# skyplane-project/skyplane

Hardware: NVIDIA H100
Metric: chunk-pipeline GB/s (raw input) (higher is better)
Workload: dtype u8/u32

## Files before the change

### skyplane_b200/csrc/md5.cuh

```cuda
#pragma once
#include <stdint.h>
#include "xxh32.cuh"
#include <type_traits>
#include <utility>

#ifndef SKY_MD5_SLOTS
#define SKY_MD5_SLOTS 4
#endif

namespace sky {

struct Md5State {
    uint32_t a, b, c, d;
};

__device__ __forceinline__ void md5_init(Md5State &s) {
    s.a = 0x67452301u;
    s.b = 0xefcdab89u;
    s.c = 0x98badcfeu;
    s.d = 0x10325476u;
}

__device__ __forceinline__ uint32_t md5_am(uint32_t a, uint32_t m, uint32_t one) {
    uint32_t r;
    asm("mad.lo.u32 %0, %1, %2, %3;" : "=r"(r) : "r"(m), "r"(one), "r"(a));
    return r;
}
__device__ __forceinline__ uint32_t md5_one() {
    uint32_t eq, lane;
    asm("mov.u32 %0, %%lanemask_eq;" : "=r"(eq));
    asm("mov.u32 %0, %%laneid;" : "=r"(lane));
    return eq >> lane;
}
#define SKY_MD5_STEP(FN, a, b, c, d, m, k, s)                      \
    {                                                              \
        uint32_t t_ = FN(b, c, d) + md5_am(a, (m), one) + (k);     \
        a = b + __funnelshift_l(t_, t_, s);                        \
    }
#define SKY_F(b, c, d) ((d) ^ ((b) & ((c) ^ (d))))
#define SKY_G(b, c, d) ((c) ^ ((d) & ((b) ^ (c))))
#define SKY_H(b, c, d) ((b) ^ (c) ^ (d))
#define SKY_I(b, c, d) ((c) ^ ((b) | ~(d)))

// ... 85 lines not shown

template <int kSlot>
__device__ __forceinline__ void cp_async_block(bool pred, uint32_t lane_ring, const uint8_t *gptr) {
    asm volatile(
        "{\n\t.reg .pred p;\n\t"
        "setp.ne.b32 p, %2, 0;\n\t"
        "@p cp.async.cg.shared.global [%0+%3], [%1], 16;\n\t"
        "@p cp.async.cg.shared.global [%0+%4], [%1+16], 16;\n\t"
        "@p cp.async.cg.shared.global [%0+%5], [%1+32], 16;\n\t"
        "@p cp.async.cg.shared.global [%0+%6], [%1+48], 16;\n\t}" ::"r"(lane_ring),
        "l"(gptr), "r"((uint32_t)pred), "n"(kSlot * 2048), "n"(kSlot * 2048 + 512), "n"(kSlot * 2048 + 1024),
        "n"(kSlot * 2048 + 1536)
        : "memory");
}
__device__ __forceinline__ void cp_async_commit() { asm volatile("cp.async.commit_group;\n" ::: "memory"); }
template <int N>
__device__ __forceinline__ void cp_async_wait() {
    asm volatile("cp.async.wait_group %0;\n" ::"n"(N) : "memory");
}

template <class F, int... I>
__device__ __forceinline__ void md5_unroll_(F &&f, std::integer_sequence<int, I...>) {
    (f(std::integral_constant<int, I>()), ...);
}
template <int N, class F>
__device__ __forceinline__ void md5_unroll(F &&f) {
    md5_unroll_(f, std::make_integer_sequence<int, N>());
}

struct Md5NoGate {
    __device__ __forceinline__ void operator()(uint64_t, bool) const {}
};

template <bool kXxh = false, class Gate = Md5NoGate>
__device__ __forceinline__ uint32_t md5_warp(uint32_t *ring, const uint8_t *src, uint64_t len, bool active, uint8_t *out,
                                             unsigned lane, Gate gate = Gate()) {
    constexpr int kSlots = SKY_MD5_SLOTS;
    static_assert(kSlots >= 2 && (kSlots & (kSlots - 1)) == 0 && 1024 % kSlots == 0, "SKY_MD5_SLOTS: a power of two, 2..1024");
    constexpr bool kGated = !std::is_same<Gate, Md5NoGate>::value;
    const uint32_t nfull = active ? (uint32_t)(len >> 6) : 0;
    const uint32_t wmax = __reduce_max_sync(0xffffffffu, nfull);
    const uint32_t trips = (wmax + (kSlots - 1)) & ~(uint32_t)(kSlots - 1);
    Md5State st;
    md5_init(st);
    Md5State fin = st;
    XxhState xs, xfin;
    if constexpr (kXxh) {
        xxh_init(xs);
        xfin = xs;
    }
    const uint32_t *lring = ring + lane * 4;
    const uint32_t lring_s = (uint32_t)__cvta_generic_to_shared(lring);
    const uint32_t one = md5_one();

    gate(0, active && len > 0);
    md5_unroll<kSlots - 1>([&](auto sc) {
        constexpr int s = decltype(sc)::value;
        cp_async_block<s>((uint32_t)s < nfull, lring_s, src + s * 64);
        cp_async_commit();
    });
    auto load_words = [&](uint32_t (&w)[16], int cs) {
#pragma unroll
        for (int q = 0; q < 4; q++) {
            const uint4 v = *reinterpret_cast<const uint4 *>(lring + (cs * 4 + q) * 128);
            w[4 * q + 0] = v.x;
            w[4 * q + 1] = v.y;
            w[4 * q + 2] = v.z;
            w[4 * q + 3] = v.w;
        }
    };
    uint32_t w[2][16];
    cp_async_wait<kSlots - 2>();
    load_words(w[0], 0);
    const uint8_t *pf_src = src + (kSlots - 1) * 64;
    auto blocks = [&](uint32_t i) {
        md5_unroll<kSlots>([&](auto uc) {
            constexpr int u = decltype(uc)::value;
            constexpr int ps = (u + kSlots - 1) & (kSlots - 1);
            constexpr int ns = (u + 1) & (kSlots - 1);
            uint32_t a = st.a, b = st.b, c = st.c, d = st.d;
            const uint32_t(&wu)[16] = w[u & 1];
            auto stripe = [&](int q) {
                if constexpr (kXxh) xxh_stripe(xs, wu[4 * q], wu[4 * q + 1], wu[4 * q + 2], wu[4 * q + 3]);
            };
            md5_round<0>(a, b, c, d, wu, one);
            stripe(0);
            cp_async_block<ps>(i + u + (kSlots - 1) < nfull, lring_s, pf_src + u * 64);
            md5_round<1>(a, b, c, d, wu, one);
            stripe(1);
            cp_async_commit();
            cp_async_wait<kSlots - 2>();
            md5_round<2>(a, b, c, d, wu, one);
            stripe(2);
            load_words(w[(u + 1) & 1], ns);
            md5_round<3>(a, b, c, d, wu, one);
            stripe(3);
            st.a += a;
            st.b += b;
            st.c += c;
            st.d += d;
            if (i + u < nfull) {
                fin = st;
                if constexpr (kXxh) xfin = xs;
            }
        });
        pf_src += kSlots * 64;
    };
    if constexpr (kGated) {
        for (uint32_t base = 0; base < trips; base += 1024) {
            gate((base >> 10) + 1, (uint64_t)(base + 1024) * 64 < len);
            const uint32_t iend = min(base + 1024, trips);
            for (uint32_t i = base; i < iend; i += kSlots) blocks(i);
        }
    } else {
        for (uint32_t i = 0; i < trips; i += kSlots) blocks(i);
    }
    cp_async_wait<0>();
    st = fin;
    uint32_t xxh = 0;
    if (active) {
        const uint32_t rem = (uint32_t)(len & 63);
        const uint8_t *tp = src + ((uint64_t)nfull << 6);
        uint32_t tw[32];
#pragma unroll
        for (int k = 0; k < 32; k++) tw[k] = 0;
        for (uint32_t k = 0; k < rem; k++) tw[k >> 2] |= (uint32_t)tp[k] << (8 * (k & 3));
        if constexpr (kXxh) {
            xs = xfin;
            const uint32_t nstripes = rem >> 4;
            for (uint32_t q = 0; q < nstripes; q++) xxh_stripe(xs, tw[4 * q], tw[4 * q + 1], tw[4 * q + 2], tw[4 * q + 3]);
            uint32_t h = xxh_merge(xs, len);
            for (uint32_t k = 4 * nstripes; k < (rem >> 2); k++) h = xxh_word(h, tw[k]);
            for (uint32_t k = rem & ~3u; k < rem; k++) h = xxh_byte(h, (tw[k >> 2] >> (8 * (k & 3))) & 0xffu);
            xxh = xxh_avalanche(h);
        }
        tw[rem >> 2] |= 0x80u << (8 * (rem & 3));
        const bool two = rem >= 56;
        const uint64_t bits = len << 3;
        tw[two ? 30 : 14] = (uint32_t)bits;
        tw[two ? 31 : 15] = (uint32_t)(bits >> 32);
        for (int t = 0; t < (two ? 2 : 1); t++) {
            uint32_t w[16];
#pragma unroll
            for (int k = 0; k < 16; k++) w[k] = tw[16 * t + k];
            md5_block(st, w, one);
        }
        uint4 dg = make_uint4(st.a, st.b, st.c, st.d);
        *reinterpret_cast<uint4 *>(out) = dg;
    }
// ... 5 lines not shown
```

### skyplane_b200/csrc/skychunk.cu

```cuda

#include <cuda_runtime.h>
#include <stdint.h>
#include <stdio.h>
#include <string.h>

#include <algorithm>
#include <memory>
#include <new>
#include <numeric>
#include <string>
#include <utility>
#include <vector>

#include "../../include/skychunk.h"
#include "frame.cuh"
#include "lz4.cuh"
#include "lz4dec.cuh"
#include "lz4hc.cuh"
#include "lz4verify.cuh"
#include "md5.cuh"
#include "secretbox.cuh"

namespace sky {

#ifndef SKY_PARSERS
#define SKY_PARSERS 12
#endif
constexpr int kParsers = SKY_PARSERS;
constexpr int kProbers = 2;
constexpr int kWarps = kProbers + kParsers;
constexpr int kThreads = kWarps * 32;
#ifndef SKY_RING_EXTRA
#define SKY_RING_EXTRA 2
#endif
constexpr int kRing = kParsers + SKY_RING_EXTRA;
constexpr int kMd5WarpsPerCta = 4;
constexpr uint32_t kRingBytes = SKY_MD5_SLOTS * 2048;
constexpr int kCtasPerSm = 2;
constexpr uint64_t kMaxChunkBlocks = 1ull << 21;

struct Ctl {
    uint64_t in_full;
    uint64_t full[kRing], empty[kRing];
    BlockDesc desc[2];
    uint32_t claim;
    volatile uint32_t block_end_seq;
    volatile uint32_t nseg;
    volatile uint32_t seg_hit[4];
    uint32_t raw, last_lits, tail_off;
    uint64_t data;
    uint32_t size;
    PendingChecksum pend;
};
constexpr uint32_t kInOff = 0;
constexpr uint32_t kTabOff = kInOff + kInBytes;
constexpr uint32_t kRingOff = kTabOff + kTableBytes;
constexpr uint32_t kRecOff = kRingOff + kRing * (uint32_t)sizeof(SegSlot);
constexpr uint32_t kPlanOff = kRecOff + kMaxSegs * (uint32_t)sizeof(SegRec);
constexpr uint32_t kCtlOff = kPlanOff + kMaxSegs * (uint32_t)sizeof(SegPlan);
constexpr uint32_t kSmemBytes = (kCtlOff + (uint32_t)sizeof(Ctl) + 127u) & ~127u;
static_assert(kSmemBytes <= 232448 / 2 - 1024, "two CTAs per SM need <= 112.5 KiB each: lower SKY_PARSERS or SKY_LZ4_ENTRIES");
static_assert(kEntries % 128 == 0, "SKY_LZ4_ENTRIES must be a multiple of 128");
static_assert(kMd5WarpsPerCta * kRingBytes <= kInBytes, "the MD5 rings live in the block buffer of a digest CTA");
static_assert(sizeof(SegSlot) % 16 == 0 && sizeof(SegRec) == 16 && sizeof(SegPlan) == 16, "layout");

template <int kId>
__device__ __forceinline__ void bar_arrive() { asm volatile("bar.arrive %0, 64;" ::"n"(kId) : "memory"); }
template <int kId>
__device__ __forceinline__ void bar_wait() { asm volatile("bar.sync %0, 64;" ::"n"(kId) : "memory"); }

template <bool kXxh, bool kBlkChk>
__device__ __forceinline__ void fused_body(const Params &p) {
    extern __shared__ __align__(128) uint8_t smem[];
    const unsigned warp = threadIdx.x >> 5, lane = threadIdx.x & 31;
    uint8_t *in = smem + kInOff;
    uint32_t *tab = reinterpret_cast<uint32_t *>(smem + kTabOff);
    SegSlot *ring = reinterpret_cast<SegSlot *>(smem + kRingOff);
    SegRec *recs = reinterpret_cast<SegRec *>(smem + kRecOff);
    SegPlan *plans = reinterpret_cast<SegPlan *>(smem + kPlanOff);
    Ctl *ctl = reinterpret_cast<Ctl *>(smem + kCtlOff);
    uint32_t smem_s = smem_u32(smem);
    asm volatile("" : "+r"(smem_s));

    const bool do_md5 = (p.flags & SKY_F_MD5) != 0, do_lz4 = (p.flags & SKY_F_LZ4) != 0;
    if (warp == 0 && lane == 0) {
        mbar_init(&ctl->in_full, 1);
        for (int i = 0; i < kRing; i++) {
            mbar_init(&ctl->full[i], 1);
            mbar_init(&ctl->empty[i], 1);
        }
        ctl->claim = 0;
        if constexpr (kBlkChk) ctl->pend.data = nullptr;
        asm volatile("fence.mbarrier_init.release.cluster;" ::: "memory");
    }
    __syncthreads();

    if (do_md5 && blockIdx.x < p.n_md5_ctas) {
        if (warp < kMd5WarpsPerCta) {
            for (uint32_t g = warp * p.n_md5_ctas + blockIdx.x; g < p.n_groups; g += p.n_md5_ctas * kMd5WarpsPerCta) {
                const uint32_t c = p.md5_order[g * 32 + lane];
                const bool active = c != 0xffffffffu;
                const uint8_t *src = nullptr;
                uint64_t len = 0;
                if (active) {
                    src = p.chunks[c].src;
                    len = p.chunks[c].len;
                }
                const uint32_t x = md5_warp<kXxh>(reinterpret_cast<uint32_t *>(in + warp * kRingBytes), src, len, active,
                                                  p.md5_out + (size_t)(active ? c : 0) * 16, lane);
                if constexpr (kXxh) {
                    if (active) p.xxh_out[c] = x;
                }
                __syncwarp();
            }
        }
        if (!do_lz4) return;
        __syncthreads();
    }
    if (!do_lz4) return;

    uint8_t *scratch = p.scratch + (size_t)blockIdx.x * kScratchBytes;
    uint32_t gseq = 0;
    uint32_t batches_done = 0;
    uint32_t my_seq = 0;
    bool have_claim = false;
    uint32_t in_phase = 0;
    constexpr unsigned kSumWarp = kWarps - 1;
    for (uint32_t it = 0;; it++) {
        BlockDesc *dsc = &ctl->desc[it & 1];
        if (warp == 0 && lane == 0) {
            claim_block(p, dsc);
            ctl->block_end_seq = 0xffffffffu;
            ctl->nseg = 0;
        }
        __syncthreads();
        if (!dsc->valid) {
            if constexpr (kBlkChk) {
                if (warp == kSumWarp) run_pending(&ctl->pend, lane);
            }
            break;
        }
        const uint8_t *src = dsc->src;
        const uint32_t L = dsc->L;

        if (warp < kProbers) {
            if (warp == 0) {
                if (lane == 0) load_block(in, src, L, &ctl->in_full);
                uint4 *t4 = reinterpret_cast<uint4 *>(tab);
                const uint4 z = make_uint4(0, 0, 0, 0);
#pragma unroll 4
                for (uint32_t k = lane; k < kEntries / 4; k += 32) t4[k] = z;
                __syncwarp();
            }
            mbar_wait(&ctl->in_full, in_phase);
            in_phase ^= 1;
            uint32_t nseg = 0;
            if (L >= kMfLimit + 1) {
                const uint32_t mflimit = L - kMfLimit;
                uint32_t seg_pos = 0, slog = 0;
                while (seg_pos <= mflimit) {
                    if (nseg >= 2) {
                        const bool h = ctl->seg_hit[(nseg - 2) & 3u] != 0u;
                        slog = h ? 0u : min(slog + 1u, kMaxStepLog);
                    }
                    const uint32_t si = gseq % kRing, ph = (gseq / kRing) & 1u;
                    SegSlot *slot = ring + si;
// ... 215 lines not shown
    p.status[c] = st;
}

struct DecRowGate {
    const uint32_t *flags;
    __device__ __forceinline__ void operator()(uint64_t row, bool wants) const {
        unsigned ns = 128;
        for (;;) {
            const bool ready = !wants || ld_relaxed32(flags + row) != 0;
            if (__all_sync(kFull, ready)) break;
            __nanosleep(ns);
            if (ns < 4096) ns <<= 1;
        }
        asm volatile("fence.acq_rel.gpu;" ::: "memory");
    }
};

__global__ void __launch_bounds__(512, 1) sky_decode_kernel(const DecParams p) {
    extern __shared__ __align__(128) uint8_t smem[];
    const unsigned warp = threadIdx.x >> 5, lane = threadIdx.x & 31;
    if (warp < kMd5WarpsPerCta) {
        const uint32_t md5_slots = gridDim.x * kMd5WarpsPerCta;
        for (uint32_t g = warp * gridDim.x + blockIdx.x; g < p.n_groups; g += md5_slots) {
            const uint32_t c = p.md5_order[g * 32 + lane];
            const bool active = c != 0xffffffffu;
            const uint8_t *src = nullptr;
            uint64_t len = 0;
            DecRowGate gate{nullptr};
            if (active) {
                src = p.chunks[c].out;
                len = p.chunks[c].raw_len;
                gate.flags = p.blk_done + p.chunks[c].blk_base;
            }
            const uint32_t x = md5_warp<true>(reinterpret_cast<uint32_t *>(smem + warp * kRingBytes), src, len, active,
                                              p.md5_out + (size_t)(active ? c : 0) * 16, lane, gate);
            if (active) {
                const int32_t s = settle_status(*reinterpret_cast<volatile int32_t *>(p.status + c));
                if (s != kDecOk) p.status[c] = s;
                else if ((p.chunks[c].checks & kChkContent) && x != p.chunks[c].content_xxh) atomicCAS(p.status + c, kDecOk, kDecChecksum);
            }
            __syncwarp();
        }
    }
    for (uint32_t c, j; claim_row_major(p.counter, p.n_chunks, p.rows, lane, c, j);) {
        const DecChunk cd = p.chunks[c];
        if (j >= cd.nblk) continue;
        int32_t st = *reinterpret_cast<volatile int32_t *>(p.status + c);
        const uint64_t pos = (uint64_t)j * kBlock;
        const uint32_t want = (uint32_t)min((uint64_t)kBlock, cd.raw_len - pos);
        if (cd.linked) {
            if (lane == 0) {
                unsigned ns = 64;
                while (ld_acquire32(p.dec_done + c) < j) {
                    __nanosleep(ns);
                    if (ns < 2048) ns <<= 1;
                }
            }
            __syncwarp();
            st = *reinterpret_cast<volatile int32_t *>(p.status + c);
        }
        if (block_may_run(st, j)) {
            const DecBlock b = p.blocks[cd.blk_base + j];
            const uint32_t sz = b.word & 0x7FFFFFFFu;
            if ((cd.checks & kChkBlock) && xxh32_warp(cd.frame + b.off, sz, lane) != b.chk) {
                st = kDecChecksum;
            } else if (b.word & 0x80000000u) {
                st = sz != want ? kDecLayout : kDecOk;
                if (st == kDecOk) warp_copy(cd.out + pos, cd.frame + b.off, sz, lane);
// ... 175 lines not shown

static thread_local std::string g_err;

#define CK(ctx, call)                                                                      \
    do {                                                                                   \
        cudaError_t e_ = (call);                                                           \
        if (e_ != cudaSuccess) {                                                           \
            char b_[512];                                                                  \
            snprintf(b_, sizeof b_, "%s -> %s (%s:%d)", #call, cudaGetErrorString(e_), __FILE__, __LINE__); \
            if (ctx) (ctx)->err = b_;                                                      \
            g_err = b_;                                                                    \
            return SKY_E_CUDA;                                                             \
        }                                                                                  \
    } while (0)

static int build_slot(sky_ctx *ctx, Slot &s, bool slabs) {
    const size_t nc = ctx->max_chunks, ng = (nc + 31) / 32 * 32;
    CK(ctx, cudaStreamCreateWithFlags(s.stream.put(), cudaStreamNonBlocking));
    CK(ctx, cudaEventCreate(s.ev_k0.put()));
    CK(ctx, cudaEventCreate(s.ev_k1.put()));
    CK(ctx, cudaEventCreate(s.ev_res.put()));
    CK(ctx, cudaEventCreateWithFlags(s.ev_h2d.put(), cudaEventDisableTiming));
    CK(ctx, cudaEventCreateWithFlags(s.ev_d2h.put(), cudaEventDisableTiming));
    BatchMeta &m = s.meta;
    CK(ctx, cudaMallocHost(m.h_desc.put(), nc * sizeof(ChunkDesc)));
    CK(ctx, cudaMalloc(m.d_desc.put(), nc * sizeof(ChunkDesc)));
    CK(ctx, cudaMallocHost(m.h_order.put(), ng * sizeof(uint32_t)));
    CK(ctx, cudaMalloc(m.d_order.put(), ng * sizeof(uint32_t)));
    CK(ctx, cudaMallocHost(m.h_chain.put(), nc * sizeof(uint64_t)));
    CK(ctx, cudaMalloc(m.d_chain.put(), nc * sizeof(uint64_t)));
    CK(ctx, m.outlen.alloc(nc));
    CK(ctx, m.md5.alloc(nc * 16));
    CK(ctx, cudaMalloc(m.xxh.put(), nc * sizeof(uint32_t)));
    CK(ctx, cudaMalloc(m.counters.put(), 64));
    CK(ctx, cudaMalloc(m.scratch.put(), (size_t)ctx->sm_count * kCtasPerSm * kScratchBytes));
    if (slabs) {
        cudaError_t e = cudaMalloc(s.d_in.put(), ctx->in_cap);
        if (e == cudaSuccess) e = cudaMalloc(s.d_out.put(), ctx->out_cap);
        if (e != cudaSuccess) { g_err = ctx->err = std::string("cudaMalloc(slab): ") + cudaGetErrorString(e); return SKY_E_NOMEM; }
    }
    return SKY_OK;
}

static int alloc_dec(sky_ctx *ctx, DecodeArrays &d) {
    if (d.d_chunks) return SKY_OK;
    const size_t nc = ctx->max_chunks;
    DecodeArrays a;
    CK(ctx, cudaMallocHost(a.h_chunks.put(), nc * sizeof(DecChunk)));
    CK(ctx, cudaMalloc(a.d_chunks.put(), nc * sizeof(DecChunk)));
    CK(ctx, cudaMallocHost(a.h_status.put(), nc * sizeof(int32_t)));
    CK(ctx, cudaMalloc(a.d_status.put(), nc * sizeof(int32_t)));
    CK(ctx, cudaMalloc(a.d_dec_done.put(), nc * sizeof(uint32_t)));
    d = std::move(a);
    return SKY_OK;
}

static int alloc_hc(sky_ctx *ctx, HcArrays &h) {
    if (h.scratch) return SKY_OK;
    HcArrays a;
    CK(ctx, cudaMalloc(a.scratch.put(), (size_t)ctx->sm_count * kHcLinkedScratchBytes));
    CK(ctx, cudaStreamCreateWithFlags(a.md5_stream.put(), cudaStreamNonBlocking));
    CK(ctx, cudaEventCreateWithFlags(a.ev_fork.put(), cudaEventDisableTiming));
    CK(ctx, cudaEventCreateWithFlags(a.ev_join.put(), cudaEventDisableTiming));
    h = std::move(a);
    return SKY_OK;
}

// ... 297 lines not shown
    (linked ? sky_verify_linked_kernel : sky_verify_kernel)<<<ctx->sm_count * 2, kVerifyThreads, 0, st>>>(p);
    CK(ctx, cudaGetLastError());
    (linked ? sky_verify_linked_settle_kernel : sky_verify_settle_kernel)<<<n, kRepairWarps * 32, 0, st>>>(p);
    CK(ctx, cudaGetLastError());
    ctx->launches += 3;
    return SKY_OK;
}

static int launch_batch(sky_ctx *ctx, Slot &s, cudaStream_t st, cudaStream_t meta_st, uint32_t n, const uint8_t *d_src,
                        const uint64_t *src_off, const uint64_t *src_len, uint8_t *d_dst, const uint64_t *dst_off, uint32_t flags) {
    if ((flags & (SKY_F_LZ4 | SKY_F_MD5)) == 0) flags |= SKY_F_LZ4 | SKY_F_MD5;
    if (flags & SKY_F_CHECKSUM) flags |= SKY_F_MD5;
    const bool xxh = (flags & SKY_F_CHECKSUM) != 0, bc = (flags & SKY_F_BLOCK_CHECKSUM) != 0;
    if (flags & SKY_F_HC) {
        const int hrc = alloc_hc(ctx, s.hc);
        if (hrc != SKY_OK) return hrc;
    }
    BatchMeta &m = s.meta;
    uint32_t rows;
    int rc = batch_geometry(n, src_len, rows, [&](uint32_t i, uint32_t nblk) {
        m.h_desc[i] = ChunkDesc{d_src + src_off[i], d_dst + dst_off[i], src_len[i], nblk};
        m.h_chain[i] = kFrameHeaderBytes;
    });
    if (rc != SKY_OK) return rc;
    const uint32_t ng = fill_md5_order(m.h_order, n, src_len);

    CK(ctx, cudaMemcpyAsync(m.d_desc, m.h_desc, n * sizeof(ChunkDesc), cudaMemcpyHostToDevice, meta_st));
    CK(ctx, cudaMemcpyAsync(m.d_order, m.h_order, ng * 32 * sizeof(uint32_t), cudaMemcpyHostToDevice, meta_st));
    CK(ctx, cudaMemcpyAsync(m.d_chain, m.h_chain, n * sizeof(uint64_t), cudaMemcpyHostToDevice, meta_st));
    if (meta_st != st) {
        CK(ctx, cudaEventRecord(s.ev_h2d, meta_st));
        CK(ctx, cudaStreamWaitEvent(st, s.ev_h2d, 0));
    }
    CK(ctx, cudaMemsetAsync(m.counters, 0, 64, st));
    memset(m.outlen.h, 0, n * sizeof(uint64_t));
    memset(m.md5.h, 0, (size_t)n * 16);

    Params p;
    p.chunks = m.d_desc;
    p.md5_order = m.d_order;
    p.chain = m.d_chain;
    p.out_len = m.outlen.d;
    p.md5_out = m.md5.d;
    p.counters = m.counters;
    p.scratch = m.scratch;
    p.n_chunks = n;
    p.n_groups = ng;
    const uint32_t grid = (uint32_t)ctx->sm_count * kCtasPerSm;
    p.n_md5_ctas = (flags & SKY_F_MD5) ? std::min(grid, std::max((ng + kMd5WarpsPerCta - 1) / kMd5WarpsPerCta,
                                                                 std::min(ng, (uint32_t)ctx->sm_count / 4))) : 0;
    p.rows = rows;
    p.flags = flags;
    p.xxh_out = m.xxh;
    CK(ctx, cudaEventRecord(s.ev_k0, st));
    if (flags & SKY_F_HC) {
        HcArrays &h = s.hc;
        const bool md5 = (flags & SKY_F_MD5) != 0;
        if (md5) {
            CK(ctx, cudaEventRecord(h.ev_fork, st));
            CK(ctx, cudaStreamWaitEvent(h.md5_stream, h.ev_fork, 0));
            Params pm = p;
            pm.flags = SKY_F_MD5;
            if (xxh) sky_fused_xxh_kernel<<<grid, kThreads, kSmemBytes, h.md5_stream>>>(pm);
            else sky_fused_kernel<<<grid, kThreads, kSmemBytes, h.md5_stream>>>(pm);
            CK(ctx, cudaGetLastError());
            CK(ctx, cudaEventRecord(h.ev_join, h.md5_stream));
            ctx->launches++;
// ... 225 lines not shown
    DecodeArrays &d = s.dec;
    uint64_t nblk_total = 0;
    uint32_t rows;
    rc = batch_geometry(n, raw_len, rows, [&](uint32_t i, uint32_t nblk) {
        d.h_chunks[i] = DecChunk{d_frames + frame_off[i], d_out + out_off[i], frame_len[i], raw_len[i], nblk_total, nblk, 0};
        nblk_total += nblk;
    });
    if (rc == SKY_OK) rc = grow_block_table(ctx, st, d.table, nblk_total + 1);
    if (rc != SKY_OK) return rc;
    BatchMeta &m = s.meta;
    CK(ctx, cudaMemcpyAsync(d.d_chunks, d.h_chunks, n * sizeof(DecChunk), cudaMemcpyHostToDevice, st));
    CK(ctx, cudaMemsetAsync(m.counters, 0, 64, st));
    CK(ctx, cudaMemsetAsync(d.d_dec_done, 0, n * sizeof(uint32_t), st));
    CK(ctx, cudaMemsetAsync(d.d_status, 0, n * sizeof(int32_t), st));
    CK(ctx, cudaMemsetAsync(d.table.done, 0, (nblk_total + 1) * sizeof(uint32_t), st));
    const uint32_t ng = fill_md5_order(m.h_order, n, raw_len);
    CK(ctx, cudaMemcpyAsync(m.d_order, m.h_order, ng * 32 * sizeof(uint32_t), cudaMemcpyHostToDevice, st));
    memset(m.md5.h, 0, (size_t)n * 16);
    DecParams p;
    p.chunks = d.d_chunks;
    p.blocks = d.table.blocks;
    p.status = d.d_status;
    p.dec_done = d.d_dec_done;
    p.counter = m.counters;
    p.blk_done = d.table.done;
    p.md5_order = m.d_order;
    p.md5_out = m.md5.d;
    p.n_chunks = n;
    p.n_groups = ng;
    p.rows = rows;
    CK(ctx, cudaEventRecord(s.ev_k0, st));
    sky_frame_index_kernel<<<(n + 127) / 128, 128, 0, st>>>(p);
    CK(ctx, cudaGetLastError());
    sky_decode_kernel<<<ctx->sm_count, 512, kMd5WarpsPerCta * kRingBytes, st>>>(p);
    CK(ctx, cudaGetLastError());
    CK(ctx, cudaEventRecord(s.ev_k1, st));
    ctx->launches += 2;
    CK(ctx, cudaMemcpyAsync(d.h_status, d.d_status, n * sizeof(int32_t), cudaMemcpyDeviceToHost, st));
    return SKY_OK;
}

int sky_decode_device(sky_ctx *ctx, uint32_t n, const void *d_frames, const uint64_t *frame_off, const uint64_t *frame_len,
                      void *d_out, const uint64_t *out_off, const uint64_t *raw_len, void *stream, int32_t *status, uint8_t *md5,
                      float *kernel_ms) {
    if (!ctx || n == 0 || !d_frames || !frame_off || !frame_len || !out_off || !raw_len) return SKY_E_INVALID;
    if (n > ctx->max_chunks) return SKY_E_CAPACITY;
    if (reinterpret_cast<uintptr_t>(d_out) & 15) return SKY_E_INVALID;
    for (uint32_t i = 0; i < n; i++) {
        if (out_off[i] & 15) return SKY_E_INVALID;
        if (raw_len[i] && !d_out) return SKY_E_INVALID;
    }
    CK(ctx, cudaSetDevice(ctx->device));
    Slot &s = ctx->slots[0];
    if (s.ticket.busy) return SKY_E_BUSY;
    cudaStream_t st = stream ? (cudaStream_t)stream : s.stream;
    int rc = launch_decode(ctx, s, st, n, (const uint8_t *)d_frames, frame_off, frame_len, (uint8_t *)d_out, out_off, raw_len);
    if (rc != SKY_OK) return rc;
    CK(ctx, cudaStreamSynchronize(st));
    if (status) memcpy(status, s.dec.h_status, n * sizeof(int32_t));
    if (md5) memcpy(md5, s.meta.md5.h, (size_t)n * 16);
    if (kernel_ms) CK(ctx, cudaEventElapsedTime(kernel_ms, s.ev_k0, s.ev_k1));
    return SKY_OK;
}

static int decode_raw(sky_ctx *ctx, Slot &s, uint32_t n, const void *const *payload, const uint64_t *payload_len, void *const *dst,
                      const uint64_t *raw_len, bool e2ee, int32_t *status, uint8_t *md5, float *kernel_ms) {
    std::vector<uint64_t> off(n), box_off(n), msg_len(payload_len, payload_len + n), md5_len(n);
// ... 53 lines not shown
    for (uint32_t i = 0; i < n; i++) {
        if (!frames[i] || (raw_len[i] && !dst[i])) return SKY_E_INVALID;
        f_off[i] = fp;
        o_off[i] = op;
        fp += round16(frame_len[i]);
        op += round16(raw_len[i]);
    }
    if (fp > ctx->out_cap || op > ctx->in_cap) return SKY_E_CAPACITY;
    if (e2ee) {
        int rc = launch_open(ctx, s, n, frames, frame_len, f_off.data(), s.d_out, f_off.data(), f_len.data());
        if (rc != SKY_OK) return rc;
    } else {
        for (uint32_t i = 0; i < n; i++)
            CK(ctx, cudaMemcpyAsync(s.d_out + f_off[i], frames[i], frame_len[i], cudaMemcpyHostToDevice, s.stream));
    }
    int rc = sky_decode_device(ctx, n, s.d_out, f_off.data(), f_len.data(), s.d_in, o_off.data(), raw_len, s.stream, status, md5, kernel_ms);
    if (rc != SKY_OK) return rc;
    if (e2ee) {
        for (uint32_t i = 0; i < n; i++)
            if (s.box.h_status[i] != 0 || frame_len[i] < (uint64_t)kBoxOverhead) {
                s.dec.h_status[i] = SKY_D_AUTH;
                if (status) status[i] = SKY_D_AUTH;
            }
    }
    for (uint32_t i = 0; i < n; i++)
        if (raw_len[i] && s.dec.h_status[i] == 0)
            CK(ctx, cudaMemcpyAsync(dst[i], s.d_in + o_off[i], raw_len[i], cudaMemcpyDeviceToHost, s.stream));
    CK(ctx, cudaStreamSynchronize(s.stream));
    return SKY_OK;
}

uint64_t sky_launch_count(const sky_ctx *ctx) { return ctx ? ctx->launches : 0; }

}
```

### skyplane_b200/native.py

```python
from __future__ import annotations

import ctypes
from pathlib import Path
from typing import Optional, Sequence

_PKG = Path(__file__).resolve().parent
LIB_PATH = _PKG / "libskychunk.so"

SKY_OK = 0
SKY_E_INVALID, SKY_E_NOGPU, SKY_E_CUDA, SKY_E_CAPACITY, SKY_E_BUSY, SKY_E_TICKET, SKY_E_NOMEM, SKY_E_NOKEY = -1, -2, -3, -4, -5, -6, -7, -8
F_LZ4, F_MD5, F_E2EE, F_HC, F_CHECKSUM, F_BLOCK_CHECKSUM = 1, 2, 16, 32, 64, 128
F_VERIFY = 1 << 12
F_LINKED = 1 << 13
CHECKSUM_BYTES = 4
BLOCK_BYTES = 65536
HC_LEVEL_SHIFT = 8
HC_LEVEL_MASK = 0xF << HC_LEVEL_SHIFT
HC_MIN_LEVEL, HC_DEFAULT_LEVEL, HC_MAX_LEVEL = 3, 5, 9
BOX_OVERHEAD = 40
D_OK, D_BAD_HEADER, D_CORRUPT, D_SIZE, D_UNSUPPORTED, D_LAYOUT, D_TRUNCATED, D_AUTH, D_CHECKSUM = 0, -1, -2, -3, -4, -5, -6, -7, -8
D_MISMATCH = -9
D_NAMES = {0: "ok", -1: "bad frame header", -2: "corrupt block", -3: "size mismatch", -4: "unsupported frame feature",
           -5: "unexpected block layout", -6: "truncated frame", -7: "box authentication failed", -8: "checksum mismatch",
           -9: "frame decodes to other bytes"}

ABI_SYMBOLS = (
    "sky_strerror", "sky_last_error", "sky_abi_version", "sky_device_count", "sky_device_pci_bus_id", "sky_kernel_config", "sky_frame_bound",
    "sky_ctx_create", "sky_ctx_destroy", "sky_pinned_alloc", "sky_pinned_free",
    "sky_submit", "sky_wait", "sky_wait_verify", "sky_set_e2ee_key", "sky_box_bound", "sky_process_device", "sky_verify_device",
    "sky_decode_device", "sky_decode",
    "sky_device_alloc", "sky_device_free", "sky_memcpy_h2d", "sky_memcpy_d2h", "sky_launch_count",
)


# ... 126 lines not shown
    if level < HC_MIN_LEVEL:
        if hc:
            raise ValueError(f"compression_level {level} is the fast compressor: the high-ratio mode takes {HC_MIN_LEVEL}..{HC_MAX_LEVEL}")
        return 0
    return hc_level_flag(level)


def frame_bound(n: int) -> int:
    return int(lib().sky_frame_bound(n))


def frame_need(n: int, checksum: bool = False, block_checksum: bool = False) -> int:
    blocks = -(-n // BLOCK_BYTES)
    return frame_bound(n) + (CHECKSUM_BYTES if checksum else 0) + (CHECKSUM_BYTES * blocks if block_checksum else 0)


_DECODE_ONLY_SUBMIT = ((F_HC, "F_HC"), (HC_LEVEL_MASK, "a high-ratio level"), (F_CHECKSUM, "F_CHECKSUM"),
                       (F_BLOCK_CHECKSUM, "F_BLOCK_CHECKSUM"), (F_VERIFY, "F_VERIFY"), (F_LINKED, "F_LINKED"))


def check_decode_flags(flags: int) -> int:
    for bit, name in _DECODE_ONLY_SUBMIT:
        if flags & bit:
            raise ValueError(f"decode does not take {name}: it is a sender option (flags {flags:#x})")
    if flags & ~(F_LZ4 | F_MD5 | F_E2EE):
        raise ValueError(f"decode does not know flag bits {flags & ~(F_LZ4 | F_MD5 | F_E2EE):#x}")
    return flags


def round16(x: int) -> int:
    return (x + 15) & ~15


def device_count() -> int:
    n = ctypes.c_int(0)
    rc = lib().sky_device_count(ctypes.byref(n))
    if rc != SKY_OK:
        return 0
    return n.value


class PinnedBuffer:

    def __init__(self, nbytes: int):
        self.nbytes = int(nbytes)
        self.addr = lib().sky_pinned_alloc(self.nbytes)
        if not self.addr:
            raise SkyChunkError(SKY_E_NOMEM, "sky_pinned_alloc failed (no CUDA device?)")
        self._arr = (ctypes.c_ubyte * max(1, self.nbytes)).from_address(self.addr)
        self.view = memoryview(self._arr).cast("B")[: self.nbytes]

    def close(self):
        if self.addr:
            self.view.release()
            del self._arr
            lib().sky_pinned_free(self.addr)
            self.addr = None

    def __del__(self):
        try:
            self.close()
        except Exception:
            pass


class Context:
# ... 46 lines not shown
        A = ctypes.c_void_p * n
        U = ctypes.c_uint64 * n
        args = (A(*src_addrs), U(*src_lens), A(*dst_addrs) if dst_addrs is not None else None, U(*dst_caps) if dst_caps is not None else None, nonces)
        if nonces is not None and len(nonces) != 24 * n:
            raise ValueError("need 24 nonce bytes per chunk")
        t = ctypes.c_uint64(0)
        self._check(lib().sky_submit(self._h, n, args[0], args[1], args[2], args[3], flags, nonces, ctypes.byref(t)))
        self._inflight[t.value] = (n, args)
        return t.value

    def wait(self, ticket: int):
        n, _keep = self._inflight.pop(ticket)
        out = (ctypes.c_uint64 * n)()
        md5 = (ctypes.c_ubyte * (16 * n))()
        ms = ctypes.c_float(0)
        self._check(lib().sky_wait(self._h, ticket, out, md5, ctypes.byref(ms)))
        raw = bytes(md5)
        return list(out), [raw[16 * i : 16 * i + 16] for i in range(n)], ms.value

    def wait_verify(self, ticket: int):
        n, _keep = self._inflight[ticket]
        out = (ctypes.c_uint64 * n)()
        md5 = (ctypes.c_ubyte * (16 * n))()
        ver = (ctypes.c_int32 * n)()
        ms = ctypes.c_float(0)
        self._check(lib().sky_wait_verify(self._h, ticket, out, md5, ver, ctypes.byref(ms)))
        del self._inflight[ticket]
        raw = bytes(md5)
        return list(out), [raw[16 * i : 16 * i + 16] for i in range(n)], list(ver), ms.value

    def process_device(self, d_src: int, src_off: Sequence[int], src_len: Sequence[int], d_dst: int, dst_off: Sequence[int],
                       dst_cap: Sequence[int], flags: int = 0, stream: int = 0):
        n = len(src_len)
        U = ctypes.c_uint64 * n
        out = U()
        md5 = (ctypes.c_ubyte * (16 * n))()
        ms = ctypes.c_float(0)
        self._check(
            lib().sky_process_device(self._h, n, d_src, U(*src_off), U(*src_len), d_dst, U(*dst_off), U(*dst_cap), flags,
                                     stream or None, out, md5, ctypes.byref(ms))
        )
        raw = bytes(md5)
        return list(out), [raw[16 * i : 16 * i + 16] for i in range(n)], ms.value

    def verify_device(self, d_src: int, src_off: Sequence[int], src_len: Sequence[int], d_frames: int, frame_off: Sequence[int],
                      frame_len: Sequence[int], frame_cap: Optional[Sequence[int]] = None, content_xxh: Optional[Sequence[int]] = None,
                      flags: int = 0, stream: int = 0):
        n = len(src_len)
        U = ctypes.c_uint64 * n
        fl = U(*frame_len)
        st = (ctypes.c_int32 * n)()
        ms = ctypes.c_float(0)
        self._check(lib().sky_verify_device(self._h, n, d_src, U(*src_off), U(*src_len), d_frames, U(*frame_off), fl,
                                            U(*frame_cap) if frame_cap is not None else None,
                                            (ctypes.c_uint32 * n)(*content_xxh) if content_xxh is not None else None, flags,
                                            stream or None, st, ctypes.byref(ms)))
        return list(st), list(fl), ms.value

    def decode_device(self, d_frames: int, frame_off: Sequence[int], frame_len: Sequence[int], d_out: int, out_off: Sequence[int],
                      raw_len: Sequence[int], stream: int = 0):
        n = len(frame_len)
        U = ctypes.c_uint64 * n
        st = (ctypes.c_int32 * n)()
        md5 = (ctypes.c_ubyte * (16 * n))()
        ms = ctypes.c_float(0)
        self._check(lib().sky_decode_device(self._h, n, d_frames, U(*frame_off), U(*frame_len), d_out, U(*out_off), U(*raw_len),
                                            stream or None, st, md5, ctypes.byref(ms)))
        raw = bytes(md5)
        return list(st), [raw[16 * i : 16 * i + 16] for i in range(n)], ms.value

    def decode(self, frame_addrs: Sequence[int], frame_lens: Sequence[int], dst_addrs: Optional[Sequence[int]], raw_lens: Sequence[int],
               flags: int = 0):
        check_decode_flags(flags)
        n = len(frame_addrs)
        A = ctypes.c_void_p * n
        U = ctypes.c_uint64 * n
# ... 30 lines not shown
```

Measured before the change: 155.9.

## Deepen MD5 cp.async ring, add chain-aware LZ4 claim throttling and tracing

Raises the default MD5 prefetch ring from 4 to 8 slots and decouples the unroll factor (fixed at 4) from ring depth, prefetching a full ring ahead with runtime slot offsets. The decode kernel keeps its own 4-slot ring. Adds a default-on SKY_CHAIN_WAIT scheme where digest CTAs publish a per-SM estimated MD5 chain end time and LZ4 claimers sleep to avoid finishing far ahead of the MD5 tail. This also grows the counters buffer. Other changes are optional trace instrumentation and Python host-side array marshaling via array.array. The added sleeping heuristic uses a hard-coded cycles-per-block constant and risks idling compressor warps.

Result: faster. 162.7 (median of 6 runs) (+4.4%).

```diff
diff --git a/skyplane_b200/csrc/md5.cuh b/skyplane_b200/csrc/md5.cuh
--- a/skyplane_b200/csrc/md5.cuh
+++ b/skyplane_b200/csrc/md5.cuh
@@ -5,10 +5,49 @@
 #include <utility>
 
 #ifndef SKY_MD5_SLOTS
-#define SKY_MD5_SLOTS 4
+#define SKY_MD5_SLOTS 8
 #endif
 
 namespace sky {
+
+#ifdef SKY_MD5_TRACE
+constexpr int kTraceGroups = 256, kTraceStamps = 512, kTraceEvery = 1024;
+struct Md5TraceStamp {
+    uint64_t t;
+    uint32_t clk;
+    uint32_t wait;
+};
+struct Md5Trace {
+    uint32_t smid, warpid, cta, stamps;
+    uint64_t t0, t1;
+    uint32_t c0, c1, wait, blocks;
+    Md5TraceStamp s[kTraceStamps];
+};
+__device__ Md5Trace g_md5_trace[kTraceGroups];
+__device__ __forceinline__ uint64_t trace_globaltimer() {
+    uint64_t t;
+    asm volatile("mov.u64 %0, %%globaltimer;" : "=l"(t));
+    return t;
+}
+__device__ __forceinline__ uint32_t trace_clock() {
+    uint32_t c;
+    asm volatile("mov.u32 %0, %%clock;" : "=r"(c));
+    return c;
+}
+__device__ __forceinline__ uint32_t trace_smid() {
+    uint32_t s;
+    asm volatile("mov.u32 %0, %%smid;" : "=r"(s));
+    return s;
+}
+__device__ __forceinline__ uint32_t trace_warpid() {
+    uint32_t w;
+    asm volatile("mov.u32 %0, %%warpid;" : "=r"(w));
+    return w;
+}
+#define SKY_MD5_TRACE_PARAM , Md5Trace *trace = nullptr
+#else
+#define SKY_MD5_TRACE_PARAM
+#endif
 
 struct Md5State {
     uint32_t a, b, c, d;
@@ -160,15 +199,16 @@
     __device__ __forceinline__ void operator()(uint64_t, bool) const {}
 };
 
-template <bool kXxh = false, class Gate = Md5NoGate>
+template <bool kXxh = false, class Gate = Md5NoGate, int kSlots = SKY_MD5_SLOTS>
 __device__ __forceinline__ uint32_t md5_warp(uint32_t *ring, const uint8_t *src, uint64_t len, bool active, uint8_t *out,
-                                             unsigned lane, Gate gate = Gate()) {
-    constexpr int kSlots = SKY_MD5_SLOTS;
-    static_assert(kSlots >= 2 && (kSlots & (kSlots - 1)) == 0 && 1024 % kSlots == 0, "SKY_MD5_SLOTS: a power of two, 2..1024");
+                                             unsigned lane, Gate gate = Gate() SKY_MD5_TRACE_PARAM) {
+    constexpr int kUnroll = 4;
+    static_assert((kSlots & (kSlots - 1)) == 0 && kSlots % kUnroll == 0 && 1024 % kSlots == 0,
+                  "the MD5 ring: a power of two, a multiple of 4 and at most 1024 blocks");
     constexpr bool kGated = !std::is_same<Gate, Md5NoGate>::value;
     const uint32_t nfull = active ? (uint32_t)(len >> 6) : 0;
     const uint32_t wmax = __reduce_max_sync(0xffffffffu, nfull);
-    const uint32_t trips = (wmax + (kSlots - 1)) & ~(uint32_t)(kSlots - 1);
+    const uint32_t trips = (wmax + (kUnroll - 1)) & ~(uint32_t)(kUnroll - 1);
     Md5State st;
     md5_init(st);
     Md5State fin = st;
@@ -180,17 +220,27 @@
     const uint32_t *lring = ring + lane * 4;
     const uint32_t lring_s = (uint32_t)__cvta_generic_to_shared(lring);
     const uint32_t one = md5_one();
+#ifdef SKY_MD5_TRACE
+    uint32_t wait_cycles = 0;
+    if (trace && lane == 0) {
+        trace->smid = trace_smid();
+        trace->warpid = trace_warpid();
+        trace->cta = blockIdx.x;
+        trace->t0 = trace_globaltimer();
+        trace->c0 = trace_clock();
+    }
+#endif
 
     gate(0, active && len > 0);
-    md5_unroll<kSlots - 1>([&](auto sc) {
+    md5_unroll<kSlots>([&](auto sc) {
         constexpr int s = decltype(sc)::value;
         cp_async_block<s>((uint32_t)s < nfull, lring_s, src + s * 64);
         cp_async_commit();
     });
-    auto load_words = [&](uint32_t (&w)[16], int cs) {
+    auto load_words = [&](uint32_t (&w)[16], uint32_t so) {
 #pragma unroll
         for (int q = 0; q < 4; q++) {
-            const uint4 v = *reinterpret_cast<const uint4 *>(lring + (cs * 4 + q) * 128);
+            const uint4 v = *reinterpret_cast<const uint4 *>(lring + so / 4 + q * 128);
             w[4 * q + 0] = v.x;
             w[4 * q + 1] = v.y;
             w[4 * q + 2] = v.z;
@@ -198,14 +248,13 @@
         }
     };
     uint32_t w[2][16];
-    cp_async_wait<kSlots - 2>();
+    cp_async_wait<kSlots - 1>();
     load_words(w[0], 0);
-    const uint8_t *pf_src = src + (kSlots - 1) * 64;
+    const uint8_t *pf_src = src + kSlots * 64;
     auto blocks = [&](uint32_t i) {
-        md5_unroll<kSlots>([&](auto uc) {
+        const uint32_t so = (i & (kSlots - 1)) * 2048, so_next = ((i + kUnroll) & (kSlots - 1)) * 2048;
+        md5_unroll<kUnroll>([&](auto uc) {
             constexpr int u = decltype(uc)::value;
-            constexpr int ps = (u + kSlots - 1) & (kSlots - 1);
-            constexpr int ns = (u + 1) & (kSlots - 1);
             uint32_t a = st.a, b = st.b, c = st.c, d = st.d;
             const uint32_t(&wu)[16] = w[u & 1];
             auto stripe = [&](int q) {
@@ -213,14 +262,20 @@
             };
             md5_round<0>(a, b, c, d, wu, one);
             stripe(0);
-            cp_async_block<ps>(i + u + (kSlots - 1) < nfull, lring_s, pf_src + u * 64);
+            cp_async_block<u>(i + u + kSlots < nfull, lring_s + so, pf_src + u * 64);
             md5_round<1>(a, b, c, d, wu, one);
             stripe(1);
             cp_async_commit();
-            cp_async_wait<kSlots - 2>();
+#ifdef SKY_MD5_TRACE
+            const uint32_t wait_from = trace_clock();
+#endif
+            cp_async_wait<kSlots - 1>();
+#ifdef SKY_MD5_TRACE
+            wait_cycles += trace_clock() - wait_from;
+#endif
             md5_round<2>(a, b, c, d, wu, one);
             stripe(2);
-            load_words(w[(u + 1) & 1], ns);
+            load_words(w[(u + 1) & 1], u + 1 < kUnroll ? so + (u + 1) * 2048 : so_next);
             md5_round<3>(a, b, c, d, wu, one);
             stripe(3);
             st.a += a;
@@ -232,17 +287,33 @@
                 if constexpr (kXxh) xfin = xs;
             }
         });
-        pf_src += kSlots * 64;
+        pf_src += kUnroll * 64;
     };
     if constexpr (kGated) {
         for (uint32_t base = 0; base < trips; base += 1024) {
             gate((base >> 10) + 1, (uint64_t)(base + 1024) * 64 < len);
             const uint32_t iend = min(base + 1024, trips);
-            for (uint32_t i = base; i < iend; i += kSlots) blocks(i);
+            for (uint32_t i = base; i < iend; i += kUnroll) blocks(i);
         }
     } else {
-        for (uint32_t i = 0; i < trips; i += kSlots) blocks(i);
-    }
+        for (uint32_t i = 0; i < trips; i += kUnroll) {
+            blocks(i);
+#ifdef SKY_MD5_TRACE
+            const uint32_t done = i + kUnroll;
+            if (trace && lane == 0 && done % kTraceEvery == 0 && done / kTraceEvery <= kTraceStamps)
+                trace->s[done / kTraceEvery - 1] = Md5TraceStamp{trace_globaltimer(), trace_clock(), wait_cycles};
+#endif
+        }
+    }
+#ifdef SKY_MD5_TRACE
+    if (trace && lane == 0) {
+        trace->t1 = trace_globaltimer();
+        trace->c1 = trace_clock();
+        trace->wait = wait_cycles;
+        trace->blocks = trips;
+        trace->stamps = min(trips / kTraceEvery, (uint32_t)kTraceStamps);
+    }
+#endif
     cp_async_wait<0>();
     st = fin;
     uint32_t xxh = 0;
diff --git a/skyplane_b200/csrc/skychunk.cu b/skyplane_b200/csrc/skychunk.cu
--- a/skyplane_b200/csrc/skychunk.cu
+++ b/skyplane_b200/csrc/skychunk.cu
@@ -36,6 +36,8 @@
 constexpr int kRing = kParsers + SKY_RING_EXTRA;
 constexpr int kMd5WarpsPerCta = 4;
 constexpr uint32_t kRingBytes = SKY_MD5_SLOTS * 2048;
+constexpr int kDecMd5Slots = 4;
+constexpr uint32_t kDecRingBytes = kDecMd5Slots * 2048;
 constexpr int kCtasPerSm = 2;
 constexpr uint64_t kMaxChunkBlocks = 1ull << 21;
 
@@ -51,6 +53,7 @@
     uint64_t data;
     uint32_t size;
     PendingChecksum pend;
+    uint64_t t0;
 };
 constexpr uint32_t kInOff = 0;
 constexpr uint32_t kTabOff = kInOff + kInBytes;
@@ -64,6 +67,51 @@
 static_assert(kMd5WarpsPerCta * kRingBytes <= kInBytes, "the MD5 rings live in the block buffer of a digest CTA");
 static_assert(sizeof(SegSlot) % 16 == 0 && sizeof(SegRec) == 16 && sizeof(SegPlan) == 16, "layout");
 
+#ifdef SKY_MD5_TRACE
+constexpr int kTraceCtas = 1024;
+struct CtaTrace {
+    uint32_t smid, digest, claims, pad;
+    uint64_t entry, first, last, exhausted;
+};
+__device__ CtaTrace g_cta_trace[kTraceCtas];
+#endif
+
+#ifndef SKY_CHAIN_WAIT
+#define SKY_CHAIN_WAIT 1
+#endif
+constexpr bool kChainWait = SKY_CHAIN_WAIT != 0;
+constexpr uint32_t kSmWords = 256;
+constexpr uint32_t kCountersBytes = 64 + kSmWords * 8;
+constexpr uint64_t kChainCyclesPerBlock = 780;
+__device__ __forceinline__ uint64_t *sm_chain_end(const Params &p) { return reinterpret_cast<uint64_t *>(p.counters + 16); }
+__device__ __forceinline__ uint32_t sm_id() {
+    uint32_t s;
+    asm volatile("mov.u32 %0, %%smid;" : "=r"(s));
+    return s;
+}
+__device__ __forceinline__ void publish_chain_end(const Params &p) {
+    uint64_t blocks = 0;
+    for (uint32_t g = blockIdx.x; g < p.n_groups; g += p.n_md5_ctas * kMd5WarpsPerCta) blocks += p.chunks[p.md5_order[g * 32]].len >> 6;
+    const uint32_t s = sm_id();
+    if (s < kSmWords)
+        atomicMax(reinterpret_cast<unsigned long long *>(sm_chain_end(p) + s), (unsigned long long)(clock64() + blocks * kChainCyclesPerBlock));
+}
+__device__ __forceinline__ void wait_for_chain(const Params &p, uint64_t t0) {
+    const uint32_t s = sm_id();
+    if (s >= kSmWords) return;
+    uint64_t end;
+    asm volatile("ld.relaxed.gpu.global.u64 %0, [%1];" : "=l"(end) : "l"(sm_chain_end(p) + s) : "memory");
+    const uint32_t total = p.rows * p.n_chunks;
+    for (;;) {
+        const uint64_t now = clock64();
+        const uint32_t w = ld_relaxed32(p.counters);
+        if (now >= end || w <= total / 64 || w >= total) return;
+        const float left = (float)(now - t0) * ((float)(total - w) / (float)w);
+        if (1.25f * left >= (float)(end - now)) return;
+        __nanosleep(10000);
+    }
+}
+
 template <int kId>
 __device__ __forceinline__ void bar_arrive() { asm volatile("bar.arrive %0, 64;" ::"n"(kId) : "memory"); }
 template <int kId>
@@ -83,6 +131,14 @@
     asm volatile("" : "+r"(smem_s));
 
     const bool do_md5 = (p.flags & SKY_F_MD5) != 0, do_lz4 = (p.flags & SKY_F_LZ4) != 0;
+#ifdef SKY_MD5_TRACE
+    CtaTrace tr{};
+    if (warp == 0 && lane == 0) {
+        tr.smid = trace_smid();
+        tr.digest = do_md5 && blockIdx.x < p.n_md5_ctas;
+        tr.entry = trace_globaltimer();
+    }
+#endif
     if (warp == 0 && lane == 0) {
         mbar_init(&ctl->in_full, 1);
         for (int i = 0; i < kRing; i++) {
@@ -90,12 +146,14 @@
             mbar_init(&ctl->empty[i], 1);
         }
         ctl->claim = 0;
+        ctl->t0 = clock64();
         if constexpr (kBlkChk) ctl->pend.data = nullptr;
         asm volatile("fence.mbarrier_init.release.cluster;" ::: "memory");
     }
     __syncthreads();
 
     if (do_md5 && blockIdx.x < p.n_md5_ctas) {
+        if (kChainWait && do_lz4 && warp == kWarps - 1 && lane == 0) publish_chain_end(p);
         if (warp < kMd5WarpsPerCta) {
             for (uint32_t g = warp * p.n_md5_ctas + blockIdx.x; g < p.n_groups; g += p.n_md5_ctas * kMd5WarpsPerCta) {
                 const uint32_t c = p.md5_order[g * 32 + lane];
@@ -107,7 +165,11 @@
                     len = p.chunks[c].len;
                 }
                 const uint32_t x = md5_warp<kXxh>(reinterpret_cast<uint32_t *>(in + warp * kRingBytes), src, len, active,
-                                                  p.md5_out + (size_t)(active ? c : 0) * 16, lane);
+                                                  p.md5_out + (size_t)(active ? c : 0) * 16, lane
+#ifdef SKY_MD5_TRACE
+                                                  , Md5NoGate(), g < kTraceGroups ? &g_md5_trace[g] : nullptr
+#endif
+                );
                 if constexpr (kXxh) {
                     if (active) p.xxh_out[c] = x;
                 }
@@ -129,9 +191,20 @@
     for (uint32_t it = 0;; it++) {
         BlockDesc *dsc = &ctl->desc[it & 1];
         if (warp == 0 && lane == 0) {
+            if (kChainWait && p.n_md5_ctas) wait_for_chain(p, ctl->t0);
             claim_block(p, dsc);
             ctl->block_end_seq = 0xffffffffu;
             ctl->nseg = 0;
+#ifdef SKY_MD5_TRACE
+            const uint64_t t = trace_globaltimer();
+            if (dsc->valid) {
+                if (tr.claims++ == 0) tr.first = t;
+                tr.last = t;
+            } else {
+                tr.exhausted = t;
+                if (blockIdx.x < kTraceCtas) g_cta_trace[blockIdx.x] = tr;
+            }
+#endif
         }
         __syncthreads();
         if (!dsc->valid) {
@@ -413,8 +486,8 @@
                 len = p.chunks[c].raw_len;
                 gate.flags = p.blk_done + p.chunks[c].blk_base;
             }
-            const uint32_t x = md5_warp<true>(reinterpret_cast<uint32_t *>(smem + warp * kRingBytes), src, len, active,
-                                              p.md5_out + (size_t)(active ? c : 0) * 16, lane, gate);
+            const uint32_t x = md5_warp<true, DecRowGate, kDecMd5Slots>(reinterpret_cast<uint32_t *>(smem + warp * kDecRingBytes), src, len,
+                                                                        active, p.md5_out + (size_t)(active ? c : 0) * 16, lane, gate);
             if (active) {
                 const int32_t s = settle_status(*reinterpret_cast<volatile int32_t *>(p.status + c));
                 if (s != kDecOk) p.status[c] = s;
@@ -656,7 +729,7 @@
     CK(ctx, m.outlen.alloc(nc));
     CK(ctx, m.md5.alloc(nc * 16));
     CK(ctx, cudaMalloc(m.xxh.put(), nc * sizeof(uint32_t)));
-    CK(ctx, cudaMalloc(m.counters.put(), 64));
+    CK(ctx, cudaMalloc(m.counters.put(), kCountersBytes));
     CK(ctx, cudaMalloc(m.scratch.put(), (size_t)ctx->sm_count * kCtasPerSm * kScratchBytes));
     if (slabs) {
         cudaError_t e = cudaMalloc(s.d_in.put(), ctx->in_cap);
@@ -1020,7 +1093,7 @@
         CK(ctx, cudaEventRecord(s.ev_h2d, meta_st));
         CK(ctx, cudaStreamWaitEvent(st, s.ev_h2d, 0));
     }
-    CK(ctx, cudaMemsetAsync(m.counters, 0, 64, st));
+    CK(ctx, cudaMemsetAsync(m.counters, 0, kCountersBytes, st));
     memset(m.outlen.h, 0, n * sizeof(uint64_t));
     memset(m.md5.h, 0, (size_t)n * 16);
 
@@ -1312,7 +1385,7 @@
     CK(ctx, cudaEventRecord(s.ev_k0, st));
     sky_frame_index_kernel<<<(n + 127) / 128, 128, 0, st>>>(p);
     CK(ctx, cudaGetLastError());
-    sky_decode_kernel<<<ctx->sm_count, 512, kMd5WarpsPerCta * kRingBytes, st>>>(p);
+    sky_decode_kernel<<<ctx->sm_count, 512, kMd5WarpsPerCta * kDecRingBytes, st>>>(p);
     CK(ctx, cudaGetLastError());
     CK(ctx, cudaEventRecord(s.ev_k1, st));
     ctx->launches += 2;
@@ -1432,4 +1505,20 @@
 
 uint64_t sky_launch_count(const sky_ctx *ctx) { return ctx ? ctx->launches : 0; }
 
-}
+#ifdef SKY_MD5_TRACE
+SKY_API int sky_md5_trace_fetch(int device, void *md5, uint64_t md5_bytes, void *ctas, uint64_t cta_bytes) {
+    if (md5_bytes != sizeof(sky::g_md5_trace) || cta_bytes != sizeof(sky::g_cta_trace)) return SKY_E_INVALID;
+    if (cudaSetDevice(device) != cudaSuccess || cudaDeviceSynchronize() != cudaSuccess ||
+        cudaMemcpyFromSymbol(md5, sky::g_md5_trace, md5_bytes) != cudaSuccess ||
+        cudaMemcpyFromSymbol(ctas, sky::g_cta_trace, cta_bytes) != cudaSuccess)
+        return SKY_E_CUDA;
+    static const char zero[sizeof(sky::g_md5_trace)] = {};
+    static_assert(sizeof(sky::g_md5_trace) >= sizeof(sky::g_cta_trace), "one zero buffer clears both");
+    if (cudaMemcpyToSymbol(sky::g_md5_trace, zero, md5_bytes) != cudaSuccess ||
+        cudaMemcpyToSymbol(sky::g_cta_trace, zero, cta_bytes) != cudaSuccess)
+        return SKY_E_CUDA;
+    return SKY_OK;
+}
+#endif
+
+}
diff --git a/skyplane_b200/native.py b/skyplane_b200/native.py
--- a/skyplane_b200/native.py
+++ b/skyplane_b200/native.py
@@ -1,5 +1,6 @@
 from __future__ import annotations
 
+import array
 import ctypes
 from pathlib import Path
 from typing import Optional, Sequence
@@ -192,6 +193,23 @@
     return (x + 15) & ~15
 
 
+def _u64_array(values: Sequence[int], n: int):
+    U = ctypes.c_uint64 * n
+    try:
+        a = array.array("Q", values)
+    except OverflowError:
+        return U(*values)
+    if len(a) > n:
+        raise IndexError("too many initializers")
+    if len(a) < n:
+        a.frombytes(bytes(8 * (n - len(a))))
+    return U.from_buffer(a)
+
+
+def _digests(raw: bytes) -> list:
+    return [raw[i : i + 16] for i in range(0, len(raw), 16)]
+
+
 def device_count() -> int:
     n = ctypes.c_int(0)
     rc = lib().sky_device_count(ctypes.byref(n))
@@ -304,16 +322,14 @@
     def process_device(self, d_src: int, src_off: Sequence[int], src_len: Sequence[int], d_dst: int, dst_off: Sequence[int],
                        dst_cap: Sequence[int], flags: int = 0, stream: int = 0):
         n = len(src_len)
-        U = ctypes.c_uint64 * n
-        out = U()
+        out = (ctypes.c_uint64 * n)()
         md5 = (ctypes.c_ubyte * (16 * n))()
         ms = ctypes.c_float(0)
         self._check(
-            lib().sky_process_device(self._h, n, d_src, U(*src_off), U(*src_len), d_dst, U(*dst_off), U(*dst_cap), flags,
-                                     stream or None, out, md5, ctypes.byref(ms))
+            lib().sky_process_device(self._h, n, d_src, _u64_array(src_off, n), _u64_array(src_len, n), d_dst, _u64_array(dst_off, n),
+                                     _u64_array(dst_cap, n), flags, stream or None, out, md5, ctypes.byref(ms))
         )
-        raw = bytes(md5)
-        return list(out), [raw[16 * i : 16 * i + 16] for i in range(n)], ms.value
+        return out[:], _digests(bytes(md5)), ms.value
 
     def verify_device(self, d_src: int, src_off: Sequence[int], src_len: Sequence[int], d_frames: int, frame_off: Sequence[int],
                       frame_len: Sequence[int], frame_cap: Optional[Sequence[int]] = None, content_xxh: Optional[Sequence[int]] = None,
```
